# KingOfTheAce2/video-restoration-pipeline-framewright

Hardware: AMD Instinct MI355X
Metric: frames/sec Real-ESRGAN x4 1080p (RRDBNet-x4plus, 1920x1080 -> 7680x4320) (higher is better)
Workload: dtype f16; 1 GPU; RealESRGAN_x4plus x4, 1920x1080 uint8 BGR frames resident in HBM -> 7680x4320 uint8 BGR in HBM, seeded synthetic weights, 43 frames per GPU

## Files before the change

video-restoration-pipeline-framewright_amd/csrc/conv3x3_wino.hip:

```cpp
#include <cstdlib>
#include <cstring>
#include <type_traits>
#include "fw_internal.h"
#include "conv_common.h"

namespace fw {

constexpr int WN_ROWP = 2 * 17 * 4;
constexpr int WN_ACT = HALO_H * WN_ROWP;
constexpr int WN_ACT_REGION = ACT_INSTR * 64;
constexpr int WN_WFR = 3 * 4 * 4;
constexpr int WN_W_REGION = WN_WFR * 64;
constexpr int WN_TOTAL = WN_ACT_REGION + 2 * WN_W_REGION;
static_assert(NWAVES == 8 && RPW == 2 && WN_TOTAL * 16 <= 160 * 1024, "written for 8 waves of 2 rows");

typedef _Float16 wn_h2 __attribute__((ext_vector_type(2)));
__device__ __forceinline__ uint4 wn_sub(uint4 a, uint4 b) {
    uint4 r;
    r.x = __builtin_bit_cast(unsigned, __builtin_bit_cast(wn_h2, a.x) - __builtin_bit_cast(wn_h2, b.x));
    r.y = __builtin_bit_cast(unsigned, __builtin_bit_cast(wn_h2, a.y) - __builtin_bit_cast(wn_h2, b.y));
    r.z = __builtin_bit_cast(unsigned, __builtin_bit_cast(wn_h2, a.z) - __builtin_bit_cast(wn_h2, b.z));
    r.w = __builtin_bit_cast(unsigned, __builtin_bit_cast(wn_h2, a.w) - __builtin_bit_cast(wn_h2, b.w));
    return r;
}
__device__ __forceinline__ uint4 wn_add(uint4 a, uint4 b) {
    uint4 r;
    r.x = __builtin_bit_cast(unsigned, __builtin_bit_cast(wn_h2, a.x) + __builtin_bit_cast(wn_h2, b.x));
    r.y = __builtin_bit_cast(unsigned, __builtin_bit_cast(wn_h2, a.y) + __builtin_bit_cast(wn_h2, b.y));
    r.z = __builtin_bit_cast(unsigned, __builtin_bit_cast(wn_h2, a.z) + __builtin_bit_cast(wn_h2, b.z));
    r.w = __builtin_bit_cast(unsigned, __builtin_bit_cast(wn_h2, a.w) + __builtin_bit_cast(wn_h2, b.w));
    return r;
}

__device__ __forceinline__ void wn_glds_w6(const void* sbase, unsigned voff, unsigned lds_piece4) {
    const unsigned long long b = (unsigned long long)sbase;
    const unsigned long long sb = ((unsigned long long)(unsigned)__builtin_amdgcn_readfirstlane((unsigned)(b >> 32)) << 32) |
                                  (unsigned long long)(unsigned)__builtin_amdgcn_readfirstlane((unsigned)b);
    lds_piece4 = __builtin_amdgcn_readfirstlane(lds_piece4);
    asm volatile(
        "s_nop 4\n\t"
        "s_mov_b32 m0, %2\n\t"
        "s_nop 0\n\t"
        "global_load_lds_dwordx4 %0, %1 offset:-4096\n\t"
        "global_load_lds_dwordx4 %0, %1 offset:-3072\n\t"
        "global_load_lds_dwordx4 %0, %1 offset:-2048\n\t"
        "global_load_lds_dwordx4 %0, %1 offset:-1024\n\t"
        "global_load_lds_dwordx4 %0, %1\n\t"
        "global_load_lds_dwordx4 %0, %1 offset:1024"
        :
        : "v"(voff), "s"(sb), "s"(lds_piece4)
        : "memory");
}

template <bool PLANES, bool STORE>
__global__ __launch_bounds__(64 * NWAVES, WAVES_PER_SIMD) void conv3x3_wino_split_kernel(const ConvParams p) {
    using T = _Float16;
    __shared__ __attribute__((aligned(16))) uint4 lds[WN_TOTAL];
    const int tid = threadIdx.x;
    const int wave = __builtin_amdgcn_readfirstlane(tid >> 6);
    const int lane = tid & 63;
    const int j = lane & 15;
    const int sl = lane >> 4;

    const int NB = gridDim.x;
    const int xcd = blockIdx.x & 7;
    const int qn = NB >> 3, rn = NB & 7;
    const int lb = (xcd < rn ? xcd * (qn + 1) : rn * (qn + 1) + (xcd - rn) * qn) + (blockIdx.x >> 3);
    const int tiles_x = (p.W + TILE_W - 1) / TILE_W;
    const int tiles_y = (p.H + TILE_H - 1) / TILE_H;
    const int ntiles = tiles_x * tiles_y;
    const int t_lo = (int)((long)lb * ntiles / NB);
    const int t_hi = (int)((long)(lb + 1) * ntiles / NB);
    if (t_lo >= t_hi) return;
    const int nch = p.cin_chunks;
    const int nitems = (t_hi - t_lo) * nch;

    unsigned relb[ACT_ITERS];
    auto piece_pos = [&](int i, int* row, int* px, int* s) {
        int idx = (ACT_ITERS * wave + i) * 64 + lane;
        if (idx >= WN_ACT) idx -= WN_ACT;
        const int rw = idx / WN_ROWP;
        const int rm = idx - rw * WN_ROWP;
        const int par = rm >= 68 ? 1 : 0;
        const int q = rm - 68 * par;
        const int ci = q >> 2;
        *row = rw;
        *px = 2 * ci + par;
        *s = (q & 3) ^ halo_swz(ci);
    };
#pragma unroll
    for (int i = 0; i < ACT_ITERS; ++i) {
        int row, px, s;
        piece_pos(i, &row, &px, &s);
        relb[i] = (unsigned)(((row * p.W + px) * p.in_cstride + s * 8) * 2) + (unsigned)(4 - i) * 1024u;
    }
    const unsigned lds_base = (unsigned)(size_t)(lds_ptr_t)lds;
    const char* in = reinterpret_cast<const char*>(p.in);
    const char* w_b = reinterpret_cast<const char*>(p.wpk);
    const unsigned lane16 = lane * 16;
    const long chunk_bytes = p.in_pstride * 2;

    unsigned a_ok = 0;
    bool a_all = true;
    const char* a_src = nullptr;
    int a_t = t_lo, a_c = 0;
    auto plan_tile = [&]() {
        int aty, atx;
        tile_pos(a_t, tiles_x, tiles_y, &aty, &atx);
        const int ty0 = aty * TILE_H, tx0 = atx * TILE_W;
        a_src = in + ((long)(ty0 - 1) * p.W + (tx0 - 1)) * p.in_cstride * 2;
        a_ok = 0;
#pragma unroll
        for (int i = 0; i < ACT_ITERS; ++i) {
            int row, px, s;
            piece_pos(i, &row, &px, &s);
            const int gy = ty0 - 1 + row, gx = tx0 - 1 + px;
            if ((unsigned)gy < (unsigned)p.H && (unsigned)gx < (unsigned)p.W) a_ok |= 1u << i;
        }
        a_all = __builtin_amdgcn_readfirstlane(__all(a_ok == (1u << ACT_ITERS) - 1u)) != 0;
    };
    auto issue_act = [&]() {
        if (a_c == 0) plan_tile();
        const unsigned dst = (unsigned)(ACT_ITERS * wave * 64);
        if (a_all) {
            glds16_batch_a(a_src, relb, lds_base + (dst + 4 * 64) * 16u);
        } else {
#pragma unroll
            for (int i = 0; i < ACT_ITERS; ++i)
                glds16_v(((a_ok >> i) & 1u) ? a_src + (relb[i] - (unsigned)(4 - i) * 1024u) : reinterpret_cast<const char*>(p.zeros),
                         lds_base + (dst + i * 64) * 16u);
        }
        if (++a_c == nch) {
            a_c = 0;
            ++a_t;
        } else {
            a_src += chunk_bytes;
        }
    };
    auto issue_w = [&](int c, int ws) {
        wn_glds_w6(w_b + (size_t)c * (WN_WFR * 1024) + (6 * wave + 4) * 1024, lane16,
                   lds_base + (unsigned)(WN_ACT_REGION + ws * WN_W_REGION + (6 * wave + 4) * 64) * 16u);
    };

    int rd[4];
#pragma unroll
    for (int k = 0; k < 4; ++k) {
        const int ci = j + (k >> 1);
        rd[k] = (k & 1) * 68 + ci * 4 + (sl ^ halo_swz(ci));
    }
    unsigned id_mask = 0;
#pragma unroll
    for (int ctl = 0; ctl < 2; ++ctl)
#pragma unroll
        for (int e = 0; e < 8; ++e)
            if (16 * ctl + j == 8 * sl + e) id_mask |= 1u << (8 * ctl + e);

    f32x4 acc[RPW][4][4];

    auto add_identity = [&](const uint4 (&xf)[RPW], float sc, int c2, auto freq_tag) {
        constexpr int F = decltype(freq_tag)::value;
#pragma unroll
        for (int ctl = 0; ctl < 2; ++ctl) {
            asm volatile("" : "+v"(sc));
            float e[8];
#pragma unroll
            for (int k = 0; k < 8; ++k) e[k] = ((id_mask >> (8 * ctl + k)) & 1u) ? sc : 0.f;
            const uint2 lo4 = Op<T>::pack4(e[0], e[1], e[2], e[3]);
            const uint2 hi4 = Op<T>::pack4(e[4], e[5], e[6], e[7]);
            const uint4 idf = make_uint4(lo4.x, lo4.y, hi4.x, hi4.y);
#pragma unroll
            for (int row = 0; row < RPW; ++row) {
                if (c2)
                    acc[row][F][2 + ctl] = Op<T>::mfma16(idf, xf[row], acc[row][F][2 + ctl]);
                else
                    acc[row][F][ctl] = Op<T>::mfma16(idf, xf[row], acc[row][F][ctl]);
            }
        }
    };

    auto add_identity1 = [&](int row, const uint4& xf, float sc, int c2, auto freq_tag) {
        constexpr int F = decltype(freq_tag)::value;
#pragma unroll
        for (int ctl = 0; ctl < 2; ++ctl) {
            asm volatile("" : "+v"(sc));
            float e[8];
#pragma unroll
            for (int k = 0; k < 8; ++k) e[k] = ((id_mask >> (8 * ctl + k)) & 1u) ? sc : 0.f;
            const uint2 lo4 = Op<T>::pack4(e[0], e[1], e[2], e[3]);
            const uint2 hi4 = Op<T>::pack4(e[4], e[5], e[6], e[7]);
            const uint4 idf = make_uint4(lo4.x, lo4.y, hi4.x, hi4.y);
            if (c2)
                acc[row][F][2 + ctl] = Op<T>::mfma16(idf, xf, acc[row][F][2 + ctl]);
            else
                acc[row][F][ctl] = Op<T>::mfma16(idf, xf, acc[row][F][ctl]);
        }
    };

    issue_w(0, 0);
    issue_act();

    int n = 0;
    for (int t = t_lo; t < t_hi; ++t) {
        int tty, ttx;
        tile_pos(t, tiles_x, tiles_y, &tty, &ttx);
        const int y0 = tty * TILE_H;
        const int x0 = ttx * TILE_W;
#pragma unroll
        for (int ct = 0; ct < 4; ++ct) {
            const f32x4 bv = *reinterpret_cast<const f32x4*>(p.bias + 16 * ct + 4 * sl);
#pragma unroll
            for (int row = 0; row < RPW; ++row) {
                acc[row][0][ct] = f32x4{0.f, 0.f, 0.f, 0.f};
                acc[row][1][ct] = bv;
                acc[row][2][ct] = f32x4{0.f, 0.f, 0.f, 0.f};
                acc[row][3][ct] = f32x4{0.f, 0.f, 0.f, 0.f};
            }
        }

        for (int c = 0; c < nch; ++c, ++n) {
            if (c > 0 || t == t_lo) FW_WAIT_VMCNT(0);
            __syncthreads();
            uint4 V[4][4];
            const bool own = !STORE && c < 2 && p.in_id_scale != 0.f;
#pragma unroll
            for (int r = 0; r < 4; ++r) {
                const uint4* row = lds + (RPW * wave + r) * WN_ROWP;
                const uint4 d0 = row[rd[0]], d1 = row[rd[1]], d2 = row[rd[2]], d3 = row[rd[3]];
                V[r][0] = wn_sub(d0, d2);
                V[r][1] = wn_add(d1, d2);
                V[r][2] = wn_sub(d2, d1);
                V[r][3] = wn_sub(d1, d3);
                if ((r == 1 || r == 2) && own) {
                    add_identity1(r - 1, d1, p.in_id_scale, c, std::integral_constant<int, 0>{});
                    add_identity1(r - 1, d2, -p.in_id_scale, c, std::integral_constant<int, 3>{});
                }
            }
            __syncthreads();
            const bool more = n + 1 < nitems;
            const int c1 = (c + 1 == nch) ? 0 : c + 1;
#ifndef FW_WN_DMA_K
#define FW_WN_DMA_K -1
#endif
            if (FW_WN_DMA_K < 0 && more) {
                issue_w(c1, (n + 1) & 1);
                issue_act();
            }
            uint4 ix0[RPW], ix1[RPW];
            const bool has_id = PLANES && c < p.n_id;
            const uint4* wl = lds + WN_ACT_REGION + (n & 1) * WN_W_REGION + lane;
#ifndef FW_WN_RING
#define FW_WN_RING 3
#endif
#ifndef FW_WN_RES_K
#define FW_WN_RES_K 17
#endif
            constexpr int RING = FW_WN_RING;
            uint4 wf[RING];
#pragma unroll
            for (int k = 0; k < RING - 1; ++k) wf[k] = wl[k * 64];
            FW_SB();
#pragma unroll
            for (int k = 0; k < WN_WFR; ++k) {
                const int dy = k / 16, f = (k / 4) & 3, ct = k & 3;
                if (k + RING - 1 < WN_WFR) wf[(k + RING - 1) % RING] = wl[(k + RING - 1) * 64];
                FW_SB();
                acc[0][f][ct] = Op<T>::mfma16(wf[k % RING], V[dy][f], acc[0][f][ct]);
                acc[1][f][ct] = Op<T>::mfma16(wf[k % RING], V[dy + 1][f], acc[1][f][ct]);
                FW_SB();
                if (k == FW_WN_DMA_K && more) {
                    issue_w(c1, (n + 1) & 1);
                    issue_act();
                    FW_SB();
                }
                if constexpr (PLANES) {
                    if (k == FW_WN_RES_K) {
                        const char* plane = reinterpret_cast<const char*>(p.in) + p.chunk_off[has_id ? c : 0];
#pragma unroll
                        for (int row = 0; row < RPW; ++row) {
                            const int y = y0 + RPW * wave + row, x = x0 + 2 * j;
                            const int cy = y < p.H ? y : p.H - 1, cx0 = x < p.W ? x : p.W - 1, cx1 = x + 1 < p.W ? x + 1 : p.W - 1;
                            const unsigned rowb = (unsigned)cy * (unsigned)p.W;
                            ix0[row] = *reinterpret_cast<const uint4*>(plane + ((rowb + cx0) * (unsigned)p.in_cstride + 8 * sl) * 2u);
                            ix1[row] = *reinterpret_cast<const uint4*>(plane + ((rowb + cx1) * (unsigned)p.in_cstride + 8 * sl) * 2u);
                        }
                        FW_SB();
                    }
                }
            }
            if constexpr (PLANES) {
                if (has_id) {
#pragma unroll
                    for (int row = 0; row < RPW; ++row) {
                        const int y = y0 + RPW * wave + row, x = x0 + 2 * j;
                        if (!(y < p.H && x < p.W)) ix0[row] = make_uint4(0, 0, 0, 0);
                        if (!(y < p.H && x + 1 < p.W)) ix1[row] = make_uint4(0, 0, 0, 0);
                    }
                    add_identity(ix0, p.id_scale[c], c & 1, std::integral_constant<int, 0>{});
                    add_identity(ix1, -p.id_scale[c], c & 1, std::integral_constant<int, 3>{});
                }
            }
        }

        FW_WAIT_VMCNT(0);
        const int ls = (sl & 1) ? 2 + (sl >> 1) : (sl >> 1);
        const int npass = (!STORE && p.out_lo) ? 2 : 1;
#pragma unroll
        for (int row = 0; row < RPW; ++row) {
            const int y = y0 + RPW * wave + row;
            if (y >= p.H) continue;
#pragma unroll
            for (int ct = 0; ct < 4; ++ct) {
                f32x4 ya = acc[row][0][ct] + acc[row][1][ct] + acc[row][2][ct];
                f32x4 yb = acc[row][1][ct] - acc[row][2][ct] - acc[row][3][ct];
                if constexpr (STORE) {
                    if (p.act == 1) {
                        ya = lrelu4(ya);
                        yb = lrelu4(yb);
                    }
                } else {
                    ya = ya * p.s1;
                    yb = yb * p.s1;
                }
                acc[row][0][ct] = ya;
                acc[row][3][ct] = yb;
            }
            for (int pass = 0; pass < npass; ++pass) {
                char* lane_base = reinterpret_cast<char*>(pass ? p.out_lo : p.out) + ((long)(2 * j) * p.out_cstride + p.out_coff + ls * 8) * 2;
                const long rowoff = ((long)y * p.W + x0) * p.out_cstride * 2;
#pragma unroll
                for (int e = 0; e < 2; ++e)
#pragma unroll
                    for (int c2 = 0; c2 < 2; ++c2) {
                        f32x4 oa = e ? acc[row][3][2 * c2] : acc[row][0][2 * c2], ob = e ? acc[row][3][2 * c2 + 1] : acc[row][0][2 * c2 + 1];
                        if (pass) {
                            oa = oa - Op<T>::unpack4(Op<T>::pack4(oa[0], oa[1], oa[2], oa[3]));
                            ob = ob - Op<T>::unpack4(Op<T>::pack4(ob[0], ob[1], ob[2], ob[3]));
                        }
                        const uint2 pa = Op<T>::pack4(oa[0], oa[1], oa[2], oa[3]);
                        const uint2 pb = Op<T>::pack4(ob[0], ob[1], ob[2], ob[3]);
                        const u32x2 sx = __builtin_amdgcn_permlane16_swap(pa.x, pb.x, false, false);
                        const u32x2 sy = __builtin_amdgcn_permlane16_swap(pa.y, pb.y, false, false);
                        if (x0 + 2 * j + e < p.W)
                            store16(lane_base + rowoff + (long)e * p.out_cstride * 2 + (long)c2 * p.out_pstride * 2, make_uint4(sx[0], sy[0], sx[1], sy[1]));
                    }
            }
        }
    }
}

#undef FW_SB

size_t pack_conv3x3_wino_weights(DType dt, const float* w, int cout, int cin, int cin_chunks, uint16_t* dst) {
    const size_t n = (size_t)cin_chunks * WN_WFR * 64 * 8;
    if (!dst) return n;
    size_t o = 0;
    for (int c = 0; c < cin_chunks; ++c)
        for (int dy = 0; dy < 3; ++dy)
            for (int f = 0; f < 4; ++f)
                for (int ct = 0; ct < 4; ++ct)
                    for (int lane = 0; lane < 64; ++lane)
                        for (int e = 0; e < 8; ++e) {
                            const int co = 16 * ct + (lane & 15), ci = 32 * c + 8 * (lane >> 4) + e;
                            float u = 0.f;
                            if (co < cout && ci < cin) {
                                const float* g = w + ((size_t)co * cin + ci) * 9 + dy * 3;
                                u = f == 0 ? g[0] : f == 1 ? 0.5f * ((g[0] + g[1]) + g[2]) : f == 2 ? 0.5f * ((g[0] - g[1]) + g[2]) : g[2];
                            }
                            dst[o++] = f32_to_operand(dt, u);
                        }
    return n;
}

void check_conv3x3_wino(const ConvParams& p, bool split) {
    if (p.H <= 0 || p.W <= 0 || p.cin_chunks <= 0 || p.upsample2x || !p.out || p.in_cstride < 32 || (p.in_cstride & 7) || (p.out_cstride & 7) ||
        (p.out_coff & 7))
        throw Error(1, "conv3x3_wino: bad problem");
    if (p.in_pstride < 32 || (p.in_pstride & 7) || (p.in_pstride == 32 && p.in_cstride < 32 * p.cin_chunks && (long)p.H * p.W > 1))
        throw Error(1, "conv3x3_wino: bad input channel/plane stride");
    if (p.out_pstride < 32 || (p.out_pstride & 7)) throw Error(1, "conv3x3_wino: bad output plane stride");
    if (p.post_act) throw Error(1, "conv3x3_wino: post_act is not implemented");
    if (p.chan_scale) throw Error(1, "conv3x3_wino: chan_scale is not implemented");
    if (p.res1 || p.res2) throw Error(1, "conv3x3_wino: fp32 residuals (res1 / res2) are not implemented");
    if (p.out_f32) throw Error(1, "conv3x3_wino: the fp32 output copy (out_f32) is not implemented");
    if (p.n_groups > 1) throw Error(1, "conv3x3_wino: output-channel groups (n_groups > 1) are not implemented");
    if (split) {
        if (p.act != 0) throw Error(1, "conv3x3_wino: no activation in the split-trunk form");
        if (p.n_id < 0 || p.n_id > 6 || p.n_id > p.cin_chunks) throw Error(1, "conv3x3_wino: bad number of residual planes (n_id)");
        if (p.n_id > 0 && (long)p.H * p.W * p.in_cstride * 2 > 0xffffffffL) throw Error(1, "conv3x3_wino: residual planes larger than 4 GiB");
        if (operand_to_f32(DT_F16, f32_to_operand(DT_F16, p.in_id_scale)) != p.in_id_scale)
            throw Error(1, "conv3x3_wino: in_id_scale not representable in f16");
        for (int i = 0; i < p.n_id; ++i)
            if (operand_to_f32(DT_F16, f32_to_operand(DT_F16, p.id_scale[i])) != p.id_scale[i])
                throw Error(1, "conv3x3_wino: identity scale not representable in f16");
    } else {
        if (p.act < 0 || p.act > 1) throw Error(1, "conv3x3_wino: act must be 0 or 1 (PReLU is not implemented)");
        if (p.n_id || p.out_lo) throw Error(1, "conv3x3_wino: residual planes / lo planes need the split-trunk form");
    }
}

void launch_conv3x3_wino_split(const ConvParams& p_in, hipStream_t stream) {
    check_conv3x3_wino(p_in, true);
    ConvParams p = p_in;
    p.zeros = conv_zero_page();
    const int tiles = ((p.W + TILE_W - 1) / TILE_W) * ((p.H + TILE_H - 1) / TILE_H);
    const int cus = conv_num_cus();
    dim3 grid(tiles < cus ? tiles : cus), block(64 * NWAVES);
    if (p.n_id > 0)
        hipLaunchKernelGGL((conv3x3_wino_split_kernel<true, false>), grid, block, 0, stream, p);
    else
        hipLaunchKernelGGL((conv3x3_wino_split_kernel<false, false>), grid, block, 0, stream, p);
    FW_HIP_CHECK(hipGetLastError());
}

void launch_conv3x3_wino_store(const ConvParams& p_in, hipStream_t stream) {
    check_conv3x3_wino(p_in, false);
    ConvParams p = p_in;
    p.zeros = conv_zero_page();
    const int tiles = ((p.W + TILE_W - 1) / TILE_W) * ((p.H + TILE_H - 1) / TILE_H);
    const int cus = conv_num_cus();
    dim3 grid(tiles < cus ? tiles : cus), block(64 * NWAVES);
    hipLaunchKernelGGL((conv3x3_wino_split_kernel<false, true>), grid, block, 0, stream, p);
    FW_HIP_CHECK(hipGetLastError());
}

}
```

video-restoration-pipeline-framewright_amd/csrc/conv3x3_pair_slide.hip:

```cpp
#include <cstdlib>
#include <type_traits>
#include "fw_internal.h"
#include "conv_common.h"

#ifndef FW_DMA_SLOT_W
#define FW_DMA_SLOT_W 2
#define FW_DMA_SLOT_A 6
#endif

namespace fw {

constexpr int PS_TH = TILE_H;
constexpr int PS_TW = TILE_W - 2;
constexpr int PS_HALO_H = TILE_H + 3;
constexpr int PS_PIECES = PS_HALO_H * ROW_PIECES;
constexpr int PS_EXTRA = PS_PIECES - ACT_ITERS * NWAVES * 64;
constexpr int PS_REGION = 41 * 64;
constexpr int PS_CARRY = 2 * ROW_PIECES;

struct SlideSmem {
    static constexpr int W_REGION = 2 * W_FRAGS * 64;
    static constexpr int W_BASE = 2 * PS_REGION;
    static constexpr int CARRY = W_BASE + 2 * W_REGION;
    static constexpr int TOTAL = CARRY + PS_CARRY;
};
static_assert(NWAVES == 8 && RPW == 2 && PS_EXTRA > 0 && PS_EXTRA <= 64, "written for 8 waves of 2 rows");
static_assert(SlideSmem::TOTAL * 16 <= 160 * 1024, "LDS");

template <typename T, bool WITH_B, typename WIdx, typename Slot>
__device__ __forceinline__ void conv_item_lag(f32x4 (&acc)[RPW][4][2], const uint4* a, const uint4* wl, const int (&rd_off)[3][2],
                                              WIdx widx, Slot dma_slot) {
    constexpr int NWU = WITH_B ? 4 : 2;
    constexpr int NK = 9 * NWU;
    constexpr int RING = 3;
    uint4 xr[5][2];
    uint4 wf[RING];
    auto tile_of = [](int w) { return WITH_B ? ((w + 2) & 3) : w; };
    auto load_w = [&](int k) {
        const int t = k / NWU, w = k - t * NWU;
        const int dx = t / 3, dy = t - 3 * dx;
        wf[k % RING] = wl[widx(dy * 3 + dx, tile_of(w)) * 64];
    };
    auto load_row = [&](int h, int dx) {
#pragma unroll
        for (int ph = 0; ph < 2; ++ph) xr[h][ph] = a[h * ROW_PIECES + rd_off[dx][ph]];
    };
#pragma unroll
    for (int h = 0; h < 5; ++h) load_row(h, 0);
#pragma unroll
    for (int k = 0; k < RING - 1; ++k) load_w(k);
    FW_SB();
#pragma unroll
    for (int t = 0; t < 9; ++t) {
        const int dx = t / 3, dy = t - 3 * dx;
        if (dx < 2 && dy == 1) load_row(0, dx + 1);
        if (dx < 2 && dy == 2) load_row(1, dx + 1);
        if (dx > 0 && dy == 0) {
            load_row(3, dx);
            load_row(4, dx);
        }
#pragma unroll
        for (int w = 0; w < NWU; ++w) {
            const int k = t * NWU + w;
            if (k + RING - 1 < NK) load_w(k + RING - 1);
            FW_SB();
            const int tile = tile_of(w);
            const int lag = tile >= 2 ? 0 : 1;
#pragma unroll
            for (int row = 0; row < RPW; ++row)
#pragma unroll
                for (int ph = 0; ph < 2; ++ph)
                    acc[row][tile][ph] = Op<T>::mfma16(wf[k % RING], xr[row + dy + lag][ph], acc[row][tile][ph]);
            FW_SB();
#pragma unroll
            for (int d = 0; d < 4 / NWU; ++d) dma_slot((t * NWU + w) * (4 / NWU) + d);
            FW_SB();
            if (dx < 2 && dy == 2 && w == (WITH_B ? 1 : 0)) load_row(2, dx + 1);
        }
    }
}

template <typename T>
__global__ __launch_bounds__(64 * NWAVES, WAVES_PER_SIMD) void conv3x3_pair_slide_kernel(const ConvPairParams p) {
    using SM = SlideSmem;
    __shared__ __attribute__((aligned(16))) uint4 lds[SM::TOTAL];
    constexpr int NW = 4;

    const int tid = threadIdx.x;
    const int wave = __builtin_amdgcn_readfirstlane(tid >> 6);
    const int lane = tid & 63;
    const int q = lane & 15;
    const int sl = lane >> 4;
    FW_STAMP_INIT();

    const int NB = gridDim.x;
    const int xcd = blockIdx.x & 7;
    const int qn = NB >> 3, rn = NB & 7;
    const int lb = (xcd < rn ? xcd * (qn + 1) : rn * (qn + 1) + (xcd - rn) * qn) + (blockIdx.x >> 3);
    const int tiles_x = (p.W + PS_TW - 1) / PS_TW;
    const int tiles_y = (p.H + PS_TH) / PS_TH;
    const int ntiles = tiles_x * tiles_y;
    const int t_lo = (int)((long)lb * ntiles / NB);
    const int t_hi = (int)((long)(lb + 1) * ntiles / NB);
    if (t_lo >= t_hi) return;
#ifdef FW_PS_NOWARM
    const int needs_warm = 0;
#else
    const int needs_warm = (t_lo % tiles_y) != 0;
#endif
    const int t_begin = t_lo - needs_warm;
    const int na = p.na;
    const int nitems = (t_hi - t_lo) * (na + 1) + needs_warm * na;

#ifndef FW_DMA_OLD_ONLY
#define FW_DMA_OLD_ONLY 0
#endif
    constexpr int NBB = FW_DMA_OLD_ONLY ? 2 : 1;
    const bool issuer = FW_DMA_OLD_ONLY ? wave < NWAVES / 2 : true;
    auto vwave = [&](int bt) { return FW_DMA_OLD_ONLY ? 2 * wave + bt : wave; };
    auto piece_idx = [&](int bt, int i) { return i < ACT_ITERS ? (ACT_ITERS * vwave(bt) + i) * 64 + lane : ACT_ITERS * NWAVES * 64 + lane; };
    unsigned relb[NBB][ACT_ITERS];
    unsigned relb_x = 0;
    auto piece_off = [&](int idx) {
        const int row = idx / ROW_PIECES;
        const int rm = idx - row * ROW_PIECES;
        const int px = rm >> 2;
        const int s = (rm & 3) ^ halo_swz(px);
        return (unsigned)(((row * p.W + px) * p.in_cstride + s * 8) * 2);
    };
#pragma unroll
    for (int bt = 0; bt < NBB; ++bt)
#pragma unroll
        for (int i = 0; i < ACT_ITERS; ++i) relb[bt][i] = piece_off(piece_idx(bt, i)) + (unsigned)(4 - i) * 1024u;
    relb_x = piece_off(piece_idx(0, ACT_ITERS));
    const bool extra_lane = wave == 0 && lane < PS_EXTRA;
    const unsigned lds_base = (unsigned)(size_t)(lds_ptr_t)lds;
    const char* in = reinterpret_cast<const char*>(p.in);
    const char* wa_b = reinterpret_cast<const char*>(p.wpk_a);
    const char* wb_b = reinterpret_cast<const char*>(p.wpk_b);
    const unsigned lane16 = lane * 16;
    const long chunk_bytes = p.in_pstride * 2;

    auto origin = [&](int t, int* R0, int* ox) {
        const int tx = t / tiles_y, ty = t - tx * tiles_y;
        *R0 = ty * PS_TH;
        *ox = tx * PS_TW - 1;
    };

    unsigned f_ok = 0;
    bool f_all = true;
    const char* f_src = nullptr;
    int f_t = t_begin, f_c = 0;
    auto plan_tile = [&]() {
        int R0, ox;
        origin(f_t, &R0, &ox);
        f_src = in + ((long)(R0 - 2) * p.W + (ox - 1)) * p.in_cstride * 2;
        f_ok = 0;
        auto inside = [&](int idx) {
            const int row = idx / ROW_PIECES;
            const int px = (idx - row * ROW_PIECES) >> 2;
            return idx < PS_PIECES && (unsigned)(R0 - 2 + row) < (unsigned)p.H && (unsigned)(ox - 1 + px) < (unsigned)p.W;
        };
#pragma unroll
        for (int bt = 0; bt < NBB; ++bt)
#pragma unroll
            for (int i = 0; i < ACT_ITERS; ++i)
                if (inside(piece_idx(bt, i))) f_ok |= 1u << (bt * ACT_ITERS + i);
        if (inside(piece_idx(0, ACT_ITERS))) f_ok |= 1u << (2 * ACT_ITERS);
        const unsigned need = ((1u << (NBB * ACT_ITERS)) - 1u) | (extra_lane ? 1u << (2 * ACT_ITERS) : 0u);
        f_all = __builtin_amdgcn_readfirstlane(__all((f_ok & need) == need)) != 0;
#ifdef FW_FORCE_SLOW_DMA
        f_all = false;
#endif
    };
    auto issue_act = [&](int stage) {
        if (f_c == 0) plan_tile();
        if (issuer) {
            const unsigned dst_x = lds_base + (unsigned)(stage * PS_REGION + ACT_ITERS * NWAVES * 64) * 16u;
#pragma unroll
            for (int bt = 0; bt < NBB; ++bt) {
                const unsigned dst = (unsigned)(stage * PS_REGION + ACT_ITERS * vwave(bt) * 64);
                if (f_all) {
                    glds16_batch_a(f_src, relb[bt], lds_base + (dst + 4 * 64) * 16u);
                } else {
#pragma unroll
                    for (int i = 0; i < ACT_ITERS; ++i)
                        glds16_v(((f_ok >> (bt * ACT_ITERS + i)) & 1u) ? f_src + (relb[bt][i] - (unsigned)(4 - i) * 1024u)
                                                                        : reinterpret_cast<const char*>(p.zeros),
                                 lds_base + (dst + i * 64) * 16u);
                }
            }
            if (extra_lane) {
                if (f_all)
                    glds16(f_src, relb_x, dst_x);
                else
                    glds16_v(((f_ok >> (2 * ACT_ITERS)) & 1u) ? f_src + relb_x : reinterpret_cast<const char*>(p.zeros), dst_x);
            }
        }
        if (++f_c == na) {
            f_c = 0;
            ++f_t;
        } else {
            f_src += chunk_bytes;
        }
    };
    auto issue_w = [&](int j, int ws) {
        if (!issuer) return;
#pragma unroll
        for (int bt = 0; bt < NBB; ++bt) {
            const int v = vwave(bt);
            const int half = v / (NWAVES / 2), k = v % (NWAVES / 2);
            if (half == 1 || j < na)
                issue_w_half((half ? wb_b : wa_b) + (size_t)j * (W_FRAGS * 1024),
                             lds_base + (unsigned)(SM::W_BASE + ws * SM::W_REGION + W_FRAGS * half * 64) * 16u, k, lane16);
        }
    };

    int rd_off[3][2];
#pragma unroll
    for (int dx = 0; dx < 3; ++dx)
#pragma unroll
        for (int ph = 0; ph < 2; ++ph) {
            const int px = 16 * ph + q + dx;
            rd_off[dx][ph] = (RPW * wave) * ROW_PIECES + px * 4 + (sl ^ halo_swz(px));
        }
    auto widx = [](int tap, int w) { return w < 2 ? tap * 2 + w : W_FRAGS + tap * 2 + (w - 2); };

    f32x4 acc[RPW][NW][2];

    const int ls = (sl & 1) ? 2 + (sl >> 1) : (sl >> 1);
    const unsigned st_off = (unsigned)((q * p.out_cstride + ls * 8) * 2);
    auto convert = [&](int w0, uint4 (&pk)[RPW][2]) {
#pragma unroll
        for (int row = 0; row < RPW; ++row)
#pragma unroll
            for (int ph = 0; ph < 2; ++ph) {
                const f32x4 va = lrelu4(w0 ? acc[row][2][ph] : acc[row][0][ph]);
                const f32x4 vb = lrelu4(w0 ? acc[row][3][ph] : acc[row][1][ph]);
                const uint2 pa = Op<T>::pack4(va[0], va[1], va[2], va[3]);
                const uint2 pb = Op<T>::pack4(vb[0], vb[1], vb[2], vb[3]);
                const u32x2 sx = __builtin_amdgcn_permlane16_swap(pa.x, pb.x, false, false);
                const u32x2 sy = __builtin_amdgcn_permlane16_swap(pa.y, pb.y, false, false);
                pk[row][ph] = make_uint4(sx[0], sy[0], sx[1], sy[1]);
            }
    };
    auto store_out = [&](const uint4 (&pk)[RPW][2], int gy0, int ox, T* plane, auto interior_tag) {
        constexpr bool INTERIOR = decltype(interior_tag)::value;
#pragma unroll
        for (int row = 0; row < RPW; ++row) {
            const int gy = gy0 + row;
            if (!INTERIOR && !((unsigned)gy < (unsigned)p.H)) continue;
            char* rowbase = reinterpret_cast<char*>(plane) + ((long)gy * p.W + ox) * p.out_cstride * 2;
#pragma unroll
            for (int ph = 0; ph < 2; ++ph) {
                const int cp = 16 * ph + q;
                if (cp >= 1 && cp <= PS_TW && (INTERIOR || (unsigned)(ox + cp) < (unsigned)p.W))
                    store16(rowbase + (long)(16 * ph) * p.out_cstride * 2 + st_off, pk[row][ph]);
            }
        }
    };
    auto write_xa = [&](const uint4 (&pk)[RPW][2], uint4* xa, int R0, int ox, auto interior_tag) {
        constexpr bool INTERIOR = decltype(interior_tag)::value;
#pragma unroll
        for (int row = 0; row < RPW; ++row) {
            const int cr = RPW * wave + row;
#pragma unroll
            for (int ph = 0; ph < 2; ++ph) {
                const int cp = 16 * ph + q, hp = cp + 1;
                uint4 v = pk[row][ph];
                if (!INTERIOR && !((unsigned)(R0 + cr) < (unsigned)p.H && (unsigned)(ox + cp) < (unsigned)p.W)) v = make_uint4(0, 0, 0, 0);
                xa[((cr + 2) * HALO_W + hp) * 4 + (ls ^ halo_swz(hp))] = v;
            }
        }
    };
    uint4* carry = lds + SM::CARRY;

    issue_w(0, 0);
    issue_act(0);

    int n = 0;
    int qd = 0;
    for (int t = t_begin; t < t_hi; ++t) {
        const bool warm = t < t_lo;
        int R0, ox;
        origin(t, &R0, &ox);
        const bool col_top = R0 == 0;
#pragma unroll
        for (int w = 0; w < NW; ++w) {
            const f32x4 bv = *reinterpret_cast<const f32x4*>((w < 2 ? p.bias_a : p.bias_b) + 16 * (w & 1) + 4 * sl);
#pragma unroll
            for (int row = 0; row < RPW; ++row)
#pragma unroll
                for (int ph = 0; ph < 2; ++ph) acc[row][w][ph] = bv;
        }
        FW_STAMP(4);
        const int ipt = warm ? na : na + 1;
        auto run_item = [&](int j, auto kind_tag, bool wait_dma) {
            constexpr int KIND = decltype(kind_tag)::value;
            constexpr bool SHARED = KIND != 2;
            FW_STAMP(SHARED ? 1 : 2);
            if (wait_dma) FW_WAIT_VMCNT(0);
            FW_STAMP(5);
            __syncthreads();
            FW_STAMP(0);
            const bool more = n + 1 < nitems;
            const int jn = (j + 1 == ipt) ? 0 : j + 1;
            const bool fetch = SHARED && more && (j + 1 < na || t + 1 < t_hi);
            const int fetch_stage = (qd + 1) & 1;
            auto dma_slot = [&](int d) {
                if (d == FW_DMA_SLOT_W) {
                    if (more) issue_w(jn, (n + 1) & 1);
                } else if (d == FW_DMA_SLOT_A) {
                    if (fetch) issue_act(fetch_stage);
                }
            };
            const uint4* a = lds + ((SHARED ? qd : qd - 1) & 1) * PS_REGION;
            const uint4* wl = lds + SM::W_BASE + (n & 1) * SM::W_REGION + lane;
            auto& slot_fn = dma_slot;
            if constexpr (KIND == 0)
                conv_item_lag<T, true>(acc, a, wl, rd_off, widx, slot_fn);
            else if constexpr (KIND == 1) {
                if (wave == NWAVES - 1) {
                    conv_item_lag<T, false>(acc, a, wl, rd_off, widx, slot_fn);
                } else {
                    slot_fn(FW_DMA_SLOT_W);
                    slot_fn(FW_DMA_SLOT_A);
                }
            }
            else
                conv_item<T, NW, 2>(acc, a, wl, rd_off, widx, slot_fn, [](const uint4 (&)[RPW][2]) {}, [](int) {});
            if (SHARED) ++qd;
            ++n;
        };
        bool wait_dma = t == t_begin;
#pragma clang loop unroll(disable)
        for (int j = 0; j < na; ++j) {
            if (warm)
                run_item(j, std::integral_constant<int, 1>{}, wait_dma);
            else
                run_item(j, std::integral_constant<int, 0>{}, wait_dma);
            wait_dma = true;
        }
        FW_STAMP(1);
        FW_WAIT_VMCNT(0);
        FW_STAMP(5);
        const bool interior = ox >= 0 && ox + TILE_W <= p.W && R0 >= 1 && R0 + TILE_H <= p.H;
        uint4 pk[RPW][2];
        if (!warm || wave == NWAVES - 1) convert(0, pk);
        if (!warm) {
            if (interior)
                store_out(pk, R0 + RPW * wave, ox, reinterpret_cast<T*>(p.out_a), std::true_type{});
            else
                store_out(pk, R0 + RPW * wave, ox, reinterpret_cast<T*>(p.out_a), std::false_type{});
        }
        FW_STAMP(6);
        __syncthreads();
        FW_STAMP(0);
        uint4* xa = lds + ((qd - 1) & 1) * PS_REGION;
        if (!warm || wave == NWAVES - 1) {
            if (interior)
                write_xa(pk, xa, R0, ox, std::true_type{});
            else
                write_xa(pk, xa, R0, ox, std::false_type{});
        }
        if (!warm) {
            if (lane < PS_CARRY / NWAVES) {
                const int i = wave * (PS_CARRY / NWAVES) + lane;
                xa[i] = col_top ? make_uint4(0, 0, 0, 0) : carry[i];
            }
            FW_STAMP(3);
            run_item(na, std::integral_constant<int, 2>{}, false);
            FW_STAMP(2);
        } else {
            __syncthreads();
            FW_STAMP(0);
        }
        if (wave == NWAVES - 1) {
#pragma unroll
            for (int k = 0; k < (PS_CARRY + 63) / 64; ++k) {
                const int i = k * 64 + lane;
                if (i < PS_CARRY) carry[i] = xa[16 * ROW_PIECES + i];
            }
        }
        FW_STAMP(3);
        if (!warm) {
            FW_WAIT_VMCNT(0);
            FW_STAMP(5);
            convert(2, pk);
            if (interior)
                store_out(pk, R0 - 1 + RPW * wave, ox, reinterpret_cast<T*>(p.out_b), std::true_type{});
            else
                store_out(pk, R0 - 1 + RPW * wave, ox, reinterpret_cast<T*>(p.out_b), std::false_type{});
            FW_STAMP(6);
        }
    }
    FW_STAMP_FLUSH(p.stamps);
}

bool pair_slide_enabled(int H, int W, int num_cus) {
    if (const char* e = getenv("FW_PAIR_SLIDE")) return atoi(e) != 0;
    const long tiles = (long)((W + PS_TW - 1) / PS_TW) * ((H + PS_TH) / PS_TH);
    return tiles >= 6L * num_cus;
}

void launch_conv3x3_pair_slide(DType dt, const ConvPairParams& p, int num_cus, hipStream_t stream) {
    const int tiles = ((p.W + PS_TW - 1) / PS_TW) * ((p.H + PS_TH) / PS_TH);
    dim3 grid(tiles < num_cus ? tiles : num_cus), block(64 * NWAVES);
    if (dt == DT_BF16)
        hipLaunchKernelGGL((conv3x3_pair_slide_kernel<__bf16>), grid, block, 0, stream, p);
    else
        hipLaunchKernelGGL((conv3x3_pair_slide_kernel<_Float16>), grid, block, 0, stream, p);
    FW_HIP_CHECK(hipGetLastError());
}

}
```

Baseline: 14.78 frames/s.

## Move identity residual adds from per-channel MFMA into spatial epilogue

Previously the residual/identity planes were added inside the channel loop by building scaled identity matrices and issuing extra MFMAs in the Winograd frequency domain, plus per-iteration global loads at a fixed k slot. Now the residual values are loaded once after the loop (two levels prefetched, a third on demand when n_id > 4) and added directly in the spatial domain after the inverse transform, using masked unpack-and-scale. This removes extra MFMAs and loads from the hot loop but adds live registers for the prefetched residuals and moves their load latency to the epilogue.

```diff
diff --git a/video-restoration-pipeline-framewright_amd/csrc/conv3x3_wino.hip b/video-restoration-pipeline-framewright_amd/csrc/conv3x3_wino.hip
--- a/video-restoration-pipeline-framewright_amd/csrc/conv3x3_wino.hip
+++ b/video-restoration-pipeline-framewright_amd/csrc/conv3x3_wino.hip
@@ -157,27 +157,6 @@
 
     f32x4 acc[RPW][4][4];
 
-    auto add_identity = [&](const uint4 (&xf)[RPW], float sc, int c2, auto freq_tag) {
-        constexpr int F = decltype(freq_tag)::value;
-#pragma unroll
-        for (int ctl = 0; ctl < 2; ++ctl) {
-            asm volatile("" : "+v"(sc));
-            float e[8];
-#pragma unroll
-            for (int k = 0; k < 8; ++k) e[k] = ((id_mask >> (8 * ctl + k)) & 1u) ? sc : 0.f;
-            const uint2 lo4 = Op<T>::pack4(e[0], e[1], e[2], e[3]);
-            const uint2 hi4 = Op<T>::pack4(e[4], e[5], e[6], e[7]);
-            const uint4 idf = make_uint4(lo4.x, lo4.y, hi4.x, hi4.y);
-#pragma unroll
-            for (int row = 0; row < RPW; ++row) {
-                if (c2)
-                    acc[row][F][2 + ctl] = Op<T>::mfma16(idf, xf[row], acc[row][F][2 + ctl]);
-                else
-                    acc[row][F][ctl] = Op<T>::mfma16(idf, xf[row], acc[row][F][ctl]);
-            }
-        }
-    };
-
     auto add_identity1 = [&](int row, const uint4& xf, float sc, int c2, auto freq_tag) {
         constexpr int F = decltype(freq_tag)::value;
 #pragma unroll
@@ -245,14 +224,9 @@
                 issue_w(c1, (n + 1) & 1);
                 issue_act();
             }
-            uint4 ix0[RPW], ix1[RPW];
-            const bool has_id = PLANES && c < p.n_id;
             const uint4* wl = lds + WN_ACT_REGION + (n & 1) * WN_W_REGION + lane;
 #ifndef FW_WN_RING
 #define FW_WN_RING 3
-#endif
-#ifndef FW_WN_RES_K
-#define FW_WN_RES_K 17
 #endif
             constexpr int RING = FW_WN_RING;
             uint4 wf[RING];
@@ -272,35 +246,52 @@
                     issue_act();
                     FW_SB();
                 }
-                if constexpr (PLANES) {
-                    if (k == FW_WN_RES_K) {
-                        const char* plane = reinterpret_cast<const char*>(p.in) + p.chunk_off[has_id ? c : 0];
-#pragma unroll
-                        for (int row = 0; row < RPW; ++row) {
-                            const int y = y0 + RPW * wave + row, x = x0 + 2 * j;
-                            const int cy = y < p.H ? y : p.H - 1, cx0 = x < p.W ? x : p.W - 1, cx1 = x + 1 < p.W ? x + 1 : p.W - 1;
-                            const unsigned rowb = (unsigned)cy * (unsigned)p.W;
-                            ix0[row] = *reinterpret_cast<const uint4*>(plane + ((rowb + cx0) * (unsigned)p.in_cstride + 8 * sl) * 2u);
-                            ix1[row] = *reinterpret_cast<const uint4*>(plane + ((rowb + cx1) * (unsigned)p.in_cstride + 8 * sl) * 2u);
-                        }
-                        FW_SB();
-                    }
-                }
-            }
-            if constexpr (PLANES) {
-                if (has_id) {
-#pragma unroll
-                    for (int row = 0; row < RPW; ++row) {
-                        const int y = y0 + RPW * wave + row, x = x0 + 2 * j;
-                        if (!(y < p.H && x < p.W)) ix0[row] = make_uint4(0, 0, 0, 0);
-                        if (!(y < p.H && x + 1 < p.W)) ix1[row] = make_uint4(0, 0, 0, 0);
-                    }
-                    add_identity(ix0, p.id_scale[c], c & 1, std::integral_constant<int, 0>{});
-                    add_identity(ix1, -p.id_scale[c], c & 1, std::integral_constant<int, 3>{});
-                }
-            }
-        }
-
+            }
+        }
+
+        uint2 rv[2][RPW][2][4];
+        int n_id = 0;
+        if constexpr (PLANES) {
+            n_id = p.n_id;
+            asm volatile("" : "+s"(n_id));
+        }
+        unsigned roff[RPW][2], rmask[RPW][2];
+        auto load_level = [&](int lv, int row, uint2 (&dst)[2][4]) {
+#pragma unroll
+            for (int h = 0; h < 2; ++h) {
+                const char* plane = reinterpret_cast<const char*>(p.in) + p.chunk_off[2 * lv + h < n_id ? 2 * lv + h : 0];
+#pragma unroll
+                for (int e = 0; e < 2; ++e)
+#pragma unroll
+                    for (int ctl = 0; ctl < 2; ++ctl)
+                        dst[e][2 * h + ctl] = *reinterpret_cast<const uint2*>(plane + (roff[row][e] + 32u * ctl));
+            }
+        };
+        auto add_level = [&](int lv, int ct, f32x4& ya, f32x4& yb, const uint2 (&src)[2][4], int row) {
+            const int i = 2 * lv + (ct >> 1);
+            const bool has = i < n_id;
+            const float sc = p.id_scale[has ? i : 0];
+            const unsigned ma = has ? rmask[row][0] : 0u, mb = has ? rmask[row][1] : 0u;
+            ya = ya + Op<T>::unpack4(make_uint2(src[0][ct].x & ma, src[0][ct].y & ma)) * sc;
+            yb = yb + Op<T>::unpack4(make_uint2(src[1][ct].x & mb, src[1][ct].y & mb)) * sc;
+        };
+        if constexpr (PLANES) {
+#pragma unroll
+            for (int row = 0; row < RPW; ++row) {
+                const int y = y0 + RPW * wave + row;
+                const unsigned rowb = (unsigned)(y < p.H ? y : p.H - 1) * (unsigned)p.W;
+#pragma unroll
+                for (int e = 0; e < 2; ++e) {
+                    const int x = x0 + 2 * j + e;
+                    roff[row][e] = ((rowb + (unsigned)(x < p.W ? x : p.W - 1)) * (unsigned)p.in_cstride + 4 * sl) * 2u;
+                    rmask[row][e] = (y < p.H && x < p.W) ? ~0u : 0u;
+                }
+            }
+#pragma unroll
+            for (int lv = 0; lv < 2; ++lv)
+#pragma unroll
+                for (int row = 0; row < RPW; ++row) load_level(lv, row, rv[lv][row]);
+        }
         FW_WAIT_VMCNT(0);
         const int ls = (sl & 1) ? 2 + (sl >> 1) : (sl >> 1);
         const int npass = (!STORE && p.out_lo) ? 2 : 1;
@@ -308,10 +299,27 @@
         for (int row = 0; row < RPW; ++row) {
             const int y = y0 + RPW * wave + row;
             if (y >= p.H) continue;
+            if constexpr (PLANES) {
+#pragma unroll
+                for (int ct = 0; ct < 4; ++ct) {
+                    FW_SB();
+                    f32x4 ya = acc[row][0][ct] + acc[row][1][ct] + acc[row][2][ct];
+                    f32x4 yb = acc[row][1][ct] - acc[row][2][ct] - acc[row][3][ct];
+                    add_level(0, ct, ya, yb, rv[0][row], row);
+                    add_level(1, ct, ya, yb, rv[1][row], row);
+                    acc[row][0][ct] = ya;
+                    acc[row][3][ct] = yb;
+                }
+                if (n_id > 4) {
+                    load_level(2, row, rv[0][row]);
+#pragma unroll
+                    for (int ct = 0; ct < 4; ++ct) add_level(2, ct, acc[row][0][ct], acc[row][3][ct], rv[0][row], row);
+                }
+            }
 #pragma unroll
             for (int ct = 0; ct < 4; ++ct) {
-                f32x4 ya = acc[row][0][ct] + acc[row][1][ct] + acc[row][2][ct];
-                f32x4 yb = acc[row][1][ct] - acc[row][2][ct] - acc[row][3][ct];
+                f32x4 ya = PLANES ? acc[row][0][ct] : acc[row][0][ct] + acc[row][1][ct] + acc[row][2][ct];
+                f32x4 yb = PLANES ? acc[row][3][ct] : acc[row][1][ct] - acc[row][2][ct] - acc[row][3][ct];
                 if constexpr (STORE) {
                     if (p.act == 1) {
                         ya = lrelu4(ya);
```

After: 14.78 frames/s. Within noise of the previous version (-0.0%).

## Replace per-block warm-up tile pass with batched 4-row carry prologue

Applied to the files above, without the earlier changes.

Blocks that start mid-column used to run a full warm-up tile through the shared pipeline, with most waves idle and only the last wave computing the carry rows. Now a dedicated prologue loads just the 4 input rows needed, batched several channel chunks at a time into the spare LDS region. Four waves compute the two carry rows with MFMA while the first tile's weights and activations are prefetched. Bias is also staged in LDS instead of reloaded from global per tile, and finer stamp categories were added for profiling. This adds prologue complexity and extra barriers in exchange for removing a mostly idle warm-up pass from the grid's critical path.

```diff
diff --git a/video-restoration-pipeline-framewright_amd/csrc/conv3x3_pair_slide.hip b/video-restoration-pipeline-framewright_amd/csrc/conv3x3_pair_slide.hip
--- a/video-restoration-pipeline-framewright_amd/csrc/conv3x3_pair_slide.hip
+++ b/video-restoration-pipeline-framewright_amd/csrc/conv3x3_pair_slide.hip
@@ -18,12 +18,39 @@
 constexpr int PS_REGION = 41 * 64;
 constexpr int PS_CARRY = 2 * ROW_PIECES;
 
+constexpr int PS_WARM_ROWS = 4;
+constexpr int PS_WARM_PIECES = PS_WARM_ROWS * ROW_PIECES;
+constexpr int PS_WARM_KIB = 9;
+constexpr int PS_WARM_SLOT = PS_WARM_KIB * 64;
+constexpr int PS_WARM_CHUNKS = 4;
+
 struct SlideSmem {
     static constexpr int W_REGION = 2 * W_FRAGS * 64;
     static constexpr int W_BASE = 2 * PS_REGION;
     static constexpr int CARRY = W_BASE + 2 * W_REGION;
-    static constexpr int TOTAL = CARRY + PS_CARRY;
+    static constexpr int BIAS = CARRY + PS_CARRY;
+    static constexpr int TOTAL = BIAS + 16;
 };
+static_assert(PS_WARM_CHUNKS * PS_WARM_SLOT <= PS_REGION && 2 * PS_WARM_CHUNKS == NWAVES, "warm-up batch: two waves per chunk slot");
+
+enum {
+    ST_BARRIER = 0, ST_SHARED = 1, ST_XA_ITEM = 2, ST_XA_LDS = 3, ST_SETUP = 4, ST_VMCNT = 5, ST_XA_EPI = 6, ST_XB_EPI = 7,
+    ST_CARRY = 8, ST_FIRST = 9, ST_W_BARRIER = 10, ST_W_MFMA = 11, ST_W_DMA = 12, ST_W_EPI = 13, ST_W_SETUP = 14, ST_LIFE = 15
+};
+#ifdef FW_PAIR_STAMP
+#undef FW_STAMP_INIT
+#undef FW_STAMP_FLUSH
+#define FW_STAMP_INIT()                                                                  \
+    unsigned long long stamp_acc[16] = {0, 0, 0, 0, 0, 0, 0, 0, 0, 0, 0, 0, 0, 0, 0, 0}; \
+    unsigned long long stamp_last = __builtin_amdgcn_s_memtime();                        \
+    const unsigned long long stamp_rt0 = __builtin_amdgcn_s_memrealtime()
+#define FW_STAMP_FLUSH(buf)                                                                                 \
+    do {                                                                                                    \
+        stamp_acc[ST_LIFE] = __builtin_amdgcn_s_memrealtime() - stamp_rt0;                                  \
+        if ((threadIdx.x & 63) == 0 && (buf))                                                               \
+            for (int k_ = 0; k_ < 16; ++k_) atomicAdd((buf) + (threadIdx.x >> 6) * 16 + k_, stamp_acc[k_]); \
+    } while (0)
+#endif
 static_assert(NWAVES == 8 && RPW == 2 && PS_EXTRA > 0 && PS_EXTRA <= 64, "written for 8 waves of 2 rows");
 static_assert(SlideSmem::TOTAL * 16 <= 160 * 1024, "LDS");
 
@@ -108,9 +135,8 @@
 #else
     const int needs_warm = (t_lo % tiles_y) != 0;
 #endif
-    const int t_begin = t_lo - needs_warm;
     const int na = p.na;
-    const int nitems = (t_hi - t_lo) * (na + 1) + needs_warm * na;
+    const int nitems = (t_hi - t_lo) * (na + 1);
 
 #ifndef FW_DMA_OLD_ONLY
 #define FW_DMA_OLD_ONLY 0
@@ -150,7 +176,7 @@
     unsigned f_ok = 0;
     bool f_all = true;
     const char* f_src = nullptr;
-    int f_t = t_begin, f_c = 0;
+    int f_t = t_lo, f_c = 0;
     auto plan_tile = [&]() {
         int R0, ox;
         origin(f_t, &R0, &ox);
@@ -204,13 +230,13 @@
             f_src += chunk_bytes;
         }
     };
-    auto issue_w = [&](int j, int ws) {
+    auto issue_w = [&](int j, int ws, int halves = 3) {
         if (!issuer) return;
 #pragma unroll
         for (int bt = 0; bt < NBB; ++bt) {
             const int v = vwave(bt);
             const int half = v / (NWAVES / 2), k = v % (NWAVES / 2);
-            if (half == 1 || j < na)
+            if (((halves >> half) & 1) && (half == 1 || j < na))
                 issue_w_half((half ? wb_b : wa_b) + (size_t)j * (W_FRAGS * 1024),
                              lds_base + (unsigned)(SM::W_BASE + ws * SM::W_REGION + W_FRAGS * half * 64) * 16u, k, lane16);
         }
@@ -274,35 +300,161 @@
         }
     };
     uint4* carry = lds + SM::CARRY;
-
-    issue_w(0, 0);
-    issue_act(0);
+    float* bias_l = reinterpret_cast<float*>(lds + SM::BIAS);
+    float bias_g = 0.f;
+    if (tid < 64) bias_g = tid < 32 ? p.bias_a[tid] : p.bias_b[tid - 32];
+
+    if (!needs_warm) {
+        issue_w(0, 0);
+        issue_act(0);
+        if (tid < 64) bias_l[tid] = bias_g;
+        __syncthreads();
+        FW_STAMP(ST_SETUP);
+    } else {
+        int R0, ox;
+        origin(t_lo, &R0, &ox);
+        const int wr0 = R0 - 3;
+        const bool w_all = R0 < p.H && ox >= 1 && ox + TILE_W < p.W;
+        const char* w_src = in + ((long)wr0 * p.W + (ox - 1)) * p.in_cstride * 2;
+        const int w_slot = wave >> 1, w_hi = wave & 1;
+        unsigned w_rel[5];
+        unsigned w_ok = 0;
+#pragma unroll
+        for (int i = 0; i < 5; ++i) {
+            const int li0 = (5 * w_hi + i) * 64 + lane;
+            const int li = li0 < PS_WARM_PIECES ? li0 : PS_WARM_PIECES - 1;
+            const int row = li / ROW_PIECES;
+            const int px = (li - row * ROW_PIECES) >> 2;
+            w_rel[i] = piece_off(li);
+            if ((unsigned)(wr0 + row) < (unsigned)p.H && (unsigned)(ox - 1 + px) < (unsigned)p.W) w_ok |= 1u << i;
+        }
+        auto warm_rows = [&](int b, int c) {
+            const char* src = w_src + (long)c * chunk_bytes;
+            const unsigned dst = lds_base + (unsigned)(PS_REGION + b * PS_WARM_SLOT + 5 * w_hi * 64) * 16u;
+            if (w_all) {
+                unsigned vo[5];
+                if (w_hi == 0) {
+#pragma unroll
+                    for (int i = 0; i < 5; ++i) vo[i] = w_rel[i] + (unsigned)(4 - i) * 1024u;
+                    glds16_batch_a(src, vo, dst + 4 * 1024u);
+                } else {
+#pragma unroll
+                    for (int i = 0; i < 4; ++i) vo[i] = w_rel[i] + (unsigned)(3 - i) * 1024u;
+                    glds16_batch_a4(src, vo, dst + 3 * 1024u);
+                }
+            } else {
+#pragma unroll
+                for (int i = 0; i < 5; ++i)
+                    if (5 * w_hi + i < PS_WARM_KIB)
+                        glds16_v(((w_ok >> i) & 1u) ? src + w_rel[i] : reinterpret_cast<const char*>(p.zeros), dst + i * 1024u);
+            }
+        };
+        auto w_slot_piece = [](int s) { return SM::W_BASE + (s < 2 ? SM::W_REGION + s * W_FRAGS * 64 : W_FRAGS * 64); };
+        const bool wb_late = na >= PS_WARM_CHUNKS;
+        const int wrow = (wave >> 1) & 1, wph = wave & 1;
+        f32x4 wacc[2] = {};
+        for (int c0 = 0; c0 < na;) {
+            const int rest = na - c0;
+            const int nb = c0 == 0 ? (rest < PS_WARM_CHUNKS ? rest : PS_WARM_CHUNKS) : (rest < 3 ? rest : 3);
+            const int wc0 = c0 == 0 ? 1 : c0;
+            const int nws = c0 == 0 ? nb - 1 : nb;
+            if (w_slot < nb) warm_rows(w_slot, c0 + w_slot);
+#pragma unroll
+            for (int s = 0; s < 3; ++s)
+                if (s < nws && (wave >> 2) == (s & 1))
+                    issue_w_half(wa_b + (size_t)(wc0 + s) * (W_FRAGS * 1024), lds_base + (unsigned)w_slot_piece(s) * 16u, wave & 3, lane16);
+            if (c0 == 0) {
+                issue_w(0, 0, wb_late ? 1 : 3);
+                if (tid < 64) bias_l[tid] = bias_g;
+            }
+            FW_STAMP(ST_W_SETUP);
+            FW_WAIT_VMCNT(0);
+            FW_STAMP(ST_W_DMA);
+            if (c0 == 0) issue_act(0);
+            __syncthreads();
+            FW_STAMP(ST_W_BARRIER);
+            if (wave >= NWAVES / 2) {
+                if (c0 == 0) {
+#pragma unroll
+                    for (int w = 0; w < 2; ++w) wacc[w] = *reinterpret_cast<const f32x4*>(bias_l + 16 * w + 4 * sl);
+                }
+                for (int b = 0; b < nb; ++b) {
+                    const uint4* xw = lds + PS_REGION + b * PS_WARM_SLOT;
+                    const uint4* wl = lds + (c0 + b == 0 ? SM::W_BASE : w_slot_piece(c0 + b - wc0)) + lane;
+#pragma unroll
+                    for (int dx = 0; dx < 3; ++dx) {
+                        const int px = 16 * wph + q + dx;
+                        const int xo = px * 4 + (sl ^ halo_swz(px));
+#pragma unroll
+                        for (int dy = 0; dy < 3; ++dy) {
+                            const uint4 xv = xw[(wrow + dy) * ROW_PIECES + xo];
+#pragma unroll
+                            for (int w = 0; w < 2; ++w)
+                                wacc[w] = Op<T>::mfma16(wl[widx(dy * 3 + dx, w) * 64], xv, wacc[w]);
+                        }
+                    }
+                }
+            }
+            FW_STAMP(ST_W_MFMA);
+            c0 += nb;
+            if (c0 < na) {
+                __syncthreads();
+                FW_STAMP(ST_W_BARRIER);
+            }
+        }
+        if (wave >= NWAVES / 2) {
+            const f32x4 va = lrelu4(wacc[0]), vb = lrelu4(wacc[1]);
+            const uint2 pa = Op<T>::pack4(va[0], va[1], va[2], va[3]);
+            const uint2 pb = Op<T>::pack4(vb[0], vb[1], vb[2], vb[3]);
+            const u32x2 sx = __builtin_amdgcn_permlane16_swap(pa.x, pb.x, false, false);
+            const u32x2 sy = __builtin_amdgcn_permlane16_swap(pa.y, pb.y, false, false);
+            uint4 v = make_uint4(sx[0], sy[0], sx[1], sy[1]);
+            const int cp = 16 * wph + q, hp = cp + 1;
+            if (!((unsigned)(R0 - 2 + wrow) < (unsigned)p.H && (unsigned)(ox + cp) < (unsigned)p.W)) v = make_uint4(0, 0, 0, 0);
+            carry[(wrow * HALO_W + hp) * 4 + (ls ^ halo_swz(hp))] = v;
+        }
+        FW_STAMP(ST_W_EPI);
+        if (wb_late) {
+            __syncthreads();
+            FW_STAMP(ST_W_BARRIER);
+            issue_w(0, 0, 2);
+            FW_STAMP(ST_W_SETUP);
+        }
+    }
 
     int n = 0;
     int qd = 0;
-    for (int t = t_begin; t < t_hi; ++t) {
-        const bool warm = t < t_lo;
+    for (int t = t_lo; t < t_hi; ++t) {
         int R0, ox;
         origin(t, &R0, &ox);
         const bool col_top = R0 == 0;
 #pragma unroll
         for (int w = 0; w < NW; ++w) {
-            const f32x4 bv = *reinterpret_cast<const f32x4*>((w < 2 ? p.bias_a : p.bias_b) + 16 * (w & 1) + 4 * sl);
+            const f32x4 bv = *reinterpret_cast<const f32x4*>(bias_l + 16 * w + 4 * sl);
 #pragma unroll
             for (int row = 0; row < RPW; ++row)
 #pragma unroll
                 for (int ph = 0; ph < 2; ++ph) acc[row][w][ph] = bv;
         }
-        FW_STAMP(4);
-        const int ipt = warm ? na : na + 1;
+        FW_STAMP(ST_SETUP);
+        const int ipt = na + 1;
         auto run_item = [&](int j, auto kind_tag, bool wait_dma) {
             constexpr int KIND = decltype(kind_tag)::value;
             constexpr bool SHARED = KIND != 2;
-            FW_STAMP(SHARED ? 1 : 2);
+            FW_STAMP(SHARED ? ST_SHARED : ST_XA_LDS);
             if (wait_dma) FW_WAIT_VMCNT(0);
-            FW_STAMP(5);
+#ifdef FW_PAIR_STAMP
+            if (j == 0) {
+                __syncthreads();
+                FW_STAMP(ST_FIRST);
+            } else {
+                FW_STAMP(ST_VMCNT);
+                __syncthreads();
+                FW_STAMP(ST_BARRIER);
+            }
+#else
             __syncthreads();
-            FW_STAMP(0);
+#endif
             const bool more = n + 1 < nitems;
             const int jn = (j + 1 == ipt) ? 0 : j + 1;
             const bool fetch = SHARED && more && (j + 1 < na || t + 1 < t_hi);
@@ -319,62 +471,41 @@
             auto& slot_fn = dma_slot;
             if constexpr (KIND == 0)
                 conv_item_lag<T, true>(acc, a, wl, rd_off, widx, slot_fn);
-            else if constexpr (KIND == 1) {
-                if (wave == NWAVES - 1) {
-                    conv_item_lag<T, false>(acc, a, wl, rd_off, widx, slot_fn);
-                } else {
-                    slot_fn(FW_DMA_SLOT_W);
-                    slot_fn(FW_DMA_SLOT_A);
-                }
-            }
             else
                 conv_item<T, NW, 2>(acc, a, wl, rd_off, widx, slot_fn, [](const uint4 (&)[RPW][2]) {}, [](int) {});
             if (SHARED) ++qd;
             ++n;
         };
-        bool wait_dma = t == t_begin;
+        bool wait_dma = t == t_lo;
 #pragma clang loop unroll(disable)
         for (int j = 0; j < na; ++j) {
-            if (warm)
-                run_item(j, std::integral_constant<int, 1>{}, wait_dma);
-            else
-                run_item(j, std::integral_constant<int, 0>{}, wait_dma);
+            run_item(j, std::integral_constant<int, 0>{}, wait_dma);
             wait_dma = true;
         }
-        FW_STAMP(1);
+        FW_STAMP(ST_SHARED);
         FW_WAIT_VMCNT(0);
-        FW_STAMP(5);
+        FW_STAMP(ST_VMCNT);
         const bool interior = ox >= 0 && ox + TILE_W <= p.W && R0 >= 1 && R0 + TILE_H <= p.H;
         uint4 pk[RPW][2];
-        if (!warm || wave == NWAVES - 1) convert(0, pk);
-        if (!warm) {
-            if (interior)
-                store_out(pk, R0 + RPW * wave, ox, reinterpret_cast<T*>(p.out_a), std::true_type{});
-            else
-                store_out(pk, R0 + RPW * wave, ox, reinterpret_cast<T*>(p.out_a), std::false_type{});
-        }
-        FW_STAMP(6);
+        convert(0, pk);
+        if (interior)
+            store_out(pk, R0 + RPW * wave, ox, reinterpret_cast<T*>(p.out_a), std::true_type{});
+        else
+            store_out(pk, R0 + RPW * wave, ox, reinterpret_cast<T*>(p.out_a), std::false_type{});
+        FW_STAMP(ST_XA_EPI);
         __syncthreads();
-        FW_STAMP(0);
+        FW_STAMP(ST_BARRIER);
         uint4* xa = lds + ((qd - 1) & 1) * PS_REGION;
-        if (!warm || wave == NWAVES - 1) {
-            if (interior)
-                write_xa(pk, xa, R0, ox, std::true_type{});
-            else
-                write_xa(pk, xa, R0, ox, std::false_type{});
-        }
-        if (!warm) {
-            if (lane < PS_CARRY / NWAVES) {
-                const int i = wave * (PS_CARRY / NWAVES) + lane;
-                xa[i] = col_top ? make_uint4(0, 0, 0, 0) : carry[i];
-            }
-            FW_STAMP(3);
-            run_item(na, std::integral_constant<int, 2>{}, false);
-            FW_STAMP(2);
-        } else {
-            __syncthreads();
-            FW_STAMP(0);
-        }
+        if (interior)
+            write_xa(pk, xa, R0, ox, std::true_type{});
+        else
+            write_xa(pk, xa, R0, ox, std::false_type{});
+        if (lane < PS_CARRY / NWAVES) {
+            const int i = wave * (PS_CARRY / NWAVES) + lane;
+            xa[i] = col_top ? make_uint4(0, 0, 0, 0) : carry[i];
+        }
+        run_item(na, std::integral_constant<int, 2>{}, false);
+        FW_STAMP(ST_XA_ITEM);
         if (wave == NWAVES - 1) {
 #pragma unroll
             for (int k = 0; k < (PS_CARRY + 63) / 64; ++k) {
@@ -382,17 +513,15 @@
                 if (i < PS_CARRY) carry[i] = xa[16 * ROW_PIECES + i];
             }
         }
-        FW_STAMP(3);
-        if (!warm) {
-            FW_WAIT_VMCNT(0);
-            FW_STAMP(5);
-            convert(2, pk);
-            if (interior)
-                store_out(pk, R0 - 1 + RPW * wave, ox, reinterpret_cast<T*>(p.out_b), std::true_type{});
-            else
-                store_out(pk, R0 - 1 + RPW * wave, ox, reinterpret_cast<T*>(p.out_b), std::false_type{});
-            FW_STAMP(6);
-        }
+        FW_STAMP(ST_CARRY);
+        FW_WAIT_VMCNT(0);
+        FW_STAMP(ST_VMCNT);
+        convert(2, pk);
+        if (interior)
+            store_out(pk, R0 - 1 + RPW * wave, ox, reinterpret_cast<T*>(p.out_b), std::true_type{});
+        else
+            store_out(pk, R0 - 1 + RPW * wave, ox, reinterpret_cast<T*>(p.out_b), std::false_type{});
+        FW_STAMP(ST_XB_EPI);
     }
     FW_STAMP_FLUSH(p.stamps);
 }
```

Result: faster. 14.45 frames/s before, 14.70 frames/s after, median of 6 (+1.7%).
